# sunchao/leveldb-rs

Measured on AMD Instinct MI355X. Metric: GiB/s device-resident batched CRC32C, 4KiB blocks; %HBM-peak at 1/2/4/8 GPUs, higher is better.
Workload: dtype u32

## Files before the change

leveldb-rs_amd/csrc/blocks.hip:

```cpp
#include <hip/hip_runtime.h>

#include <algorithm>
#include <string>

#include "lvh.h"

namespace lvk {

template <int G, bool STRIDED>
__global__ __launch_bounds__(kThreads) void crc32c_batch_kernel(Params P, const uint4 *__restrict__ image) {
    if (static_cast<uint64_t>(blockIdx.x) * kWaves * (64 / G) >= P.n) return;
    stage_tables(image);
    const uint32_t lane = threadIdx.x & 63u;
    const uint32_t wave = threadIdx.x >> 6;
    const Lut L = make_lut(lane);
    constexpr uint32_t kGroups = 64 / G;
    const uint64_t gid = (static_cast<uint64_t>(blockIdx.x) * kWaves + wave) * kGroups + lane / G;
    const uint64_t gstride = static_cast<uint64_t>(gridDim.x) * kWaves * kGroups;
    group_stream<G, STRIDED>(P, gid, gstride, lane % G, L);
}

constexpr uint32_t kFuseMax = 16;

__device__ __forceinline__ void fuse_pieces(const Params &P, const uint32_t *fm, uint32_t (&res)[kWaves][64],
                                            uint32_t lane, uint32_t wave) {
    __syncthreads();
    if (wave != 0) return;
    const uint32_t s = 1u << P.pshift;
    const uint64_t v = static_cast<uint64_t>(blockIdx.x) * 64u + lane;
    const uint32_t k = lane & (s - 1u);
    uint32_t acc = v < P.n ? gf2_apply(fm + (s - 1u - k) * 33u, res[lane >> 2][lane & 3u]) : 0u;
    for (uint32_t d = s >> 1; d >= 1; d >>= 1) acc ^= __shfl_xor(acc, d);
    if (v < P.n && k == 0) P.out[v >> P.pshift] = final_crc(P, acc);
}
static_assert(kFuseMax * 33 <= kWaves * 64, "fused combine matrices fit g_oidx");
template <int G, bool SEEDED, bool PIECES = false, bool FUSE = false, bool GATHER = false>
__global__ __launch_bounds__(kThreads) void crc32c_blocks_kernel(Params P, uint32_t nb,
                                                                 const uint4 *__restrict__ image) {
    static_assert(!FUSE || (PIECES && G == 16), "fused combine: pieces of the G = 16 kernel");
    const uint32_t lane = threadIdx.x & 63u;
    const uint32_t wave = __builtin_amdgcn_readfirstlane(threadIdx.x >> 6);
    constexpr uint32_t kGroups = 64 / G;
    constexpr uint64_t kRow = 16ull * G;
    constexpr uint64_t kBatch = kRow * U;
    const uint32_t gl = lane % G;
    constexpr uint32_t kW = kWaves;
    uint64_t blk = (static_cast<uint64_t>(blockIdx.x) * kW + wave) * kGroups + lane / G;
    const uint64_t gstride = static_cast<uint64_t>(gridDim.x) * kW * kGroups;
    const uint64_t wblk0 = (static_cast<uint64_t>(blockIdx.x) * kW + wave) * kGroups;
    const uint64_t pmask = (1ull << P.pshift) - 1;
    auto block_off = [&](uint64_t k) -> uint64_t {
        const uint64_t kk = k < P.n ? k : 0;
        const uint64_t b = PIECES ? kk >> P.pshift : kk;
        if constexpr (GATHER) return P.off[b];
        return b * P.stride;
    };
    auto report = [&](uint32_t bad) {
        if constexpr (GATHER)
            if (bad && P.herr) atomicOr(P.herr, bad);
    };
    auto block_at = [&](uint64_t k, uint64_t bo) {
        const uint64_t kk = k < P.n ? k : 0;
        if constexpr (GATHER) bo &= ~static_cast<uint64_t>(15);
        if constexpr (PIECES) return P.base + bo + (kk & pmask) * P.plen + 16u * gl;
        return P.base + bo + 16u * gl;
    };
    auto block_ptr = [&](uint64_t k) { return block_at(k, block_off(k)); };
    auto seed_ld = [&](uint64_t k) -> uint32_t {
        const uint64_t kk = k < P.n ? k : 0;
        if constexpr (PIECES) {
            const uint32_t sd = SEEDED ? ~P.seed[kk >> P.pshift] : 0xffffffffu;
            return (kk & pmask) ? 0u : sd;
        }
        return ~P.seed[kk];
    };
    constexpr bool kVarS0 = SEEDED || PIECES;

    const uint64_t o0 = block_off(blk);
    uint64_t ptr = block_at(blk, o0);
    uint64_t o1 = GATHER ? block_off(blk + gstride) : 0;
    uint64_t o2 = o1;
    uint32_t s0 = kVarS0 ? seed_ld(blk) : 0xffffffffu;
    uint32_t s0n = s0;
    uint4 slot0[U], slot1[U];
#pragma unroll
    for (uint32_t i = 0; i < U; ++i) slot0[i] = load16(ptr + kRow * i);
    const uint64_t nblk = PIECES ? (P.n >> P.pshift) : P.n;
    const uint64_t lstr = static_cast<uint64_t>(gridDim.x) * kThreads;
    const uint64_t lb0 = static_cast<uint64_t>(blockIdx.x) * kThreads + threadIdx.x;
    uint32_t lq[4] = {0, 0, 0, 0};
    const bool lcheck = GATHER && P.herr;
    if (lcheck) {
#pragma unroll
        for (uint32_t i = 0; i < 4; ++i) {
            const uint64_t b = lb0 + i * lstr;
            lq[i] = b < nblk ? P.len[b] ^ P.hlen : 0u;
        }
    }
    uint32_t *const fm = &g_oidx[0][0];
    if constexpr (FUSE) {
        const uint32_t nw = (1u << P.pshift) * 32u;
        for (uint32_t i = threadIdx.x; i < nw; i += kThreads) fm[(i >> 5) * 33 + (i & 31u)] = P.mats[i];
    }
    stage_tables(image);
    uint32_t lbad = lq[0] | lq[1] | lq[2] | lq[3];
    if (lcheck)
        for (uint64_t b = lb0 + 4 * lstr; b < nblk; b += lstr) lbad |= P.len[b] ^ P.hlen;
    if constexpr (GATHER) report(((o0 & 15u) ? LV_HINT_ERR_MISALIGNED : 0u) | (lbad ? LV_HINT_ERR_NOT_UNIFORM : 0u));
    if (wblk0 >= P.n) {
        if constexpr (FUSE) fuse_pieces(P, fm, g_ocrc, lane, wave);
        return;
    }
    if constexpr (PIECES) {
        if (nb <= U && (FUSE || wblk0 + gstride >= P.n)) {
            uint4 v1[U], v2[U], v3[U];
#pragma unroll
            for (uint32_t i = 0; i < U; ++i) {
                v1[i] = load16(ptr + kBatch * (nb > 1 ? 1u : 0u) + kRow * i);
                v2[i] = load16(ptr + kBatch * (nb > 2 ? 2u : 0u) + kRow * i);
                v3[i] = load16(ptr + kBatch * (nb > 3 ? 3u : 0u) + kRow * i);
            }
            const Lut L = make_lut(lane);
            uint32_t A[U] = {};
            if (gl == 0) slot0[0].x ^= kVarS0 ? seed_ld(blk) : 0xffffffffu;
            fold_batch_carry(slot0, A, L, nb == 1);
            if (nb > 1) fold_batch_carry(v1, A, L, nb == 2);
            if (nb > 2) fold_batch_carry(v2, A, L, nb == 3);
            if (nb > 3) fold_batch_carry(v3, A, L, nb == 4);
            const uint32_t X = merge_group<G, -1, -1, true>(A, L);
            if constexpr (FUSE) {
                if (gl == 0) g_ocrc[wave][lane / G] = X;
                fuse_pieces(P, fm, g_ocrc, lane, wave);
            } else {
                if (gl == 0 && blk < P.n) P.out[blk] = X;
            }
            return;
        }
    }
    const uint64_t rounds = (P.n - 1 - wblk0) / gstride + 1;
    if (G == 16 && nb >= 8 && rounds * nb >= 64)
        for (uint32_t k = 0; k < wave * LVK_STAGGER; ++k) __builtin_amdgcn_s_sleep(32);
    const Lut L = make_lut(lane);
    uint32_t A[U] = {};
    uint32_t st_val = 0;
    uint64_t st_ptr = 0;

    auto step = [&](uint64_t r, uint32_t j, uint4(&cur)[U], uint4(&nxt)[U]) {
        const bool lastj = j + 1 == nb;
        const bool more = !lastj || r + 1 < rounds;
        if constexpr (GATHER) o2 = block_off(blk + 2 * gstride);
        const uint64_t nptr = lastj ? (GATHER ? block_at(blk + gstride, o1) : block_ptr(blk + gstride)) : ptr + kBatch;
        const uint64_t lptr = more ? nptr : GATHER ? ptr : P.base + 16u * gl;
        if constexpr (kVarS0) s0n = seed_ld(blk + gstride);
#pragma unroll
        for (uint32_t i = 0; i < U; ++i) nxt[i] = load16(lptr + kRow * i);
        if (j == 0 && gl == 0) cur[0].x ^= s0;
        fold_batch_carry(cur, A, L, lastj);
        if (lastj) {
            const uint32_t X = merge_group<G, -1, -1, true>(A, L);
#pragma unroll
            for (uint32_t i = 0; i < U; ++i) A[i] = 0u;
            if (gl == 0) g_ocrc[wave][(r % G) * kGroups + lane / G] = PIECES ? X : final_crc(P, X);
            if (!FUSE && ((r + 1) % G == 0 || r + 1 == rounds)) {
                __builtin_amdgcn_wave_barrier();
                const uint64_t r0 = r - r % G;
                const uint64_t k = wblk0 + (r0 + lane / kGroups) * gstride + lane % kGroups;
                st_val = g_ocrc[wave][lane];
                st_ptr = reinterpret_cast<uint64_t>(P.out + (k < P.n ? k : 0));
                if (lane < (r - r0 + 1) * kGroups && k < P.n) *reinterpret_cast<uint32_t *>(st_ptr) = st_val;
                __builtin_amdgcn_wave_barrier();
            }
            blk += gstride;
            if constexpr (kVarS0) s0 = s0n;
            if constexpr (GATHER) {
                if (o1 & 15u) report(LV_HINT_ERR_MISALIGNED);
                o1 = o2;
            }
        }
        ptr = nptr;
    };

    const uint64_t total = rounds * nb;
    uint64_t t = 0;
    uint64_t r = 0;
    uint32_t j = 0;
    for (;;) {
        step(r, j, slot0, slot1);
        if (++t == total) break;
        if (++j == nb) { j = 0; ++r; }
        step(r, j, slot1, slot0);
        if (++t == total) break;
        if (++j == nb) { j = 0; ++r; }
    }
    asm volatile("" ::"v"(st_val), "v"(st_ptr));
    if constexpr (FUSE) fuse_pieces(P, fm, g_ocrc, lane, wave);
}

__global__ __launch_bounds__(256) void combine_pieces_kernel(const uint32_t *__restrict__ raw, uint64_t n, uint32_t s,
                                                             const uint32_t *__restrict__ mats,
                                                             uint32_t *__restrict__ out, uint32_t flags) {
    __shared__ uint32_t M[65 * 33];
    for (uint32_t i = threadIdx.x; i < 65 * 32; i += blockDim.x) M[(i >> 5) * 33 + (i & 31u)] = mats[i];
    __syncthreads();
    const uint32_t lane = threadIdx.x & 63u;
    const uint32_t w = s < 64 ? s : 64, reps = s <= 64 ? 1 : s / 64;
    const uint64_t nw = static_cast<uint64_t>(gridDim.x) * (blockDim.x / 64);
    for (uint64_t b = static_cast<uint64_t>(blockIdx.x) * (blockDim.x / 64) + (threadIdx.x >> 6); b < n; b += nw) {
        uint32_t acc = 0;
        if (lane < w) {
            uint32_t nx = raw[b * s + lane];
            for (uint32_t m = 0; m < reps; ++m) {
                const uint32_t cur = nx;
                if (m + 1 < reps) nx = raw[b * s + lane + 64 * (m + 1)];
                acc = (m ? gf2_apply(M + 64 * 33, acc) : 0u) ^ cur;
            }
            acc = gf2_apply(M + (w - 1 - lane) * 33, acc);
        }
#pragma unroll
        for (int k = 32; k >= 1; k >>= 1) acc ^= __shfl_xor(acc, k);
        if (lane == 0) {
            const uint32_t crc = ~acc;
            out[b] = (flags & LV_CRC_MASK) ? mask_crc(crc) : crc;
        }
    }
}

__global__ __launch_bounds__(1024) void combine_pieces_wg_kernel(const uint32_t *__restrict__ raw, uint32_t s,
                                                                 const uint32_t *__restrict__ tabs,
                                                                 uint32_t *__restrict__ out, uint32_t flags) {
    __shared__ __attribute__((aligned(16))) uint32_t T[11 * 1024];
    __shared__ uint32_t part[16];
    const uint32_t c = s / 1024u;
    const uint32_t lc = c >= 4u ? 2u : 1u;
    stage_words(T, tabs, 256u);
    stage_words(T + 1024, tabs + lc * 1024u, 10u * 256u);
    __syncthreads();
    const uint32_t t = threadIdx.x, lane = t & 63u, w = t >> 6;
    const uint64_t b = blockIdx.x;
    uint32_t acc = 0;
    for (uint32_t i = 0; i < c; ++i) acc = (i ? tab_shift(T, acc) : 0u) ^ raw[b * s + t * c + i];
#pragma unroll
    for (uint32_t u = 0; u < 6; ++u) {
        const uint32_t right = __shfl_down(acc, 1u << u);
        const uint32_t sh = tab_shift(T + (1u + u) * 1024u, acc);
        if ((lane & ((2u << u) - 1u)) == 0) acc = sh ^ right;
    }
    if (lane == 0) part[w] = acc;
    __syncthreads();
    if (w == 0) {
        acc = lane < 16u ? part[lane] : 0u;
#pragma unroll
        for (uint32_t u = 0; u < 4; ++u) {
            const uint32_t right = __shfl_down(acc, 1u << u);
            const uint32_t sh = tab_shift(T + (7u + u) * 1024u, acc);
            if ((lane & ((2u << u) - 1u)) == 0) acc = sh ^ right;
        }
        if (lane == 0) {
            const uint32_t crc = ~acc;
            out[b] = (flags & LV_CRC_MASK) ? mask_crc(crc) : crc;
        }
    }
}

}

namespace lvh {

template <int G, bool STRIDED>
void launch_one(const DevCtx &c, int gi, const uint8_t *arena, const uint64_t *off,
                const uint32_t *len, uint64_t stride, uint32_t blen, const uint32_t *seed,
                uint32_t *out, uint64_t n, uint32_t flags, hipStream_t s) {
    const uint64_t groups_per_wg = static_cast<uint64_t>(lvk::kWaves) * (64 / G);
    uint64_t grid = (n + groups_per_wg - 1) / groups_per_wg;
    if (grid > static_cast<uint64_t>(c.cus)) grid = c.cus;
    if (grid == 0) grid = 1;
    lvk::Params P{};
    P.base = reinterpret_cast<uint64_t>(arena);
    P.off = off;
    P.len = len;
    P.seed = seed;
    P.out = out;
    P.n = n;
    P.stride = stride;
    P.blen = blen;
    P.flags = flags;
    P.ent = nullptr;
    P.sseed = nullptr;
    static const std::string name = std::string("crc32c_batch_kernel<") + std::to_string(G) +
                                    (STRIDED ? ",strided>" : ",offsets>");
    g_kernel = name.c_str();
    hipLaunchKernelGGL((lvk::crc32c_batch_kernel<G, STRIDED>), dim3(static_cast<uint32_t>(grid)),
                       dim3(lvk::kThreads), 0, s, P, c.image[gi]);
}

template <bool STRIDED>
void launch_g(const DevCtx &c, int gi, const uint8_t *arena, const uint64_t *off,
              const uint32_t *len, uint64_t stride, uint32_t blen, const uint32_t *seed,
              uint32_t *out, uint64_t n, uint32_t flags, hipStream_t s) {
    switch (gi) {
        case 0: launch_one<1, STRIDED>(c, gi, arena, off, len, stride, blen, seed, out, n, flags, s); break;
        case 1: launch_one<4, STRIDED>(c, gi, arena, off, len, stride, blen, seed, out, n, flags, s); break;
        case 2: launch_one<16, STRIDED>(c, gi, arena, off, len, stride, blen, seed, out, n, flags, s); break;
        default: launch_one<64, STRIDED>(c, gi, arena, off, len, stride, blen, seed, out, n, flags, s); break;
    }
}

void launch_group(const DevCtx &c, bool strided, int gi, const uint8_t *arena, const uint64_t *off,
                  const uint32_t *len, uint64_t stride, uint32_t blen, const uint32_t *seed, uint32_t *out, uint64_t n,
                  uint32_t flags, hipStream_t s) {
    if (strided)
        launch_g<true>(c, gi, arena, off, len, stride, blen, seed, out, n, flags, s);
    else
// ... 194 lines not shown
```

leveldb-rs_amd/csrc/context.hip:

```cpp
#include <hip/hip_runtime.h>

#include <algorithm>
#include <cstring>
#include <thread>

#include "../../include/lvgpu/crc32c.h"
#include "crc32c_gf2.h"
#include "lvh.h"

namespace lvk {

__device__ __forceinline__ uint64_t splitmix64(uint64_t x) {
    x += 0x9E3779B97F4A7C15ull;
    x = (x ^ (x >> 30)) * 0xBF58476D1CE4E5B9ull;
    x = (x ^ (x >> 27)) * 0x94D049BB133111EBull;
    return x ^ (x >> 31);
}

__global__ void fill_words_kernel(uint64_t *dst, uint64_t word0, uint64_t nwords, uint64_t seed) {
    for (uint64_t i = blockIdx.x * 256ull + threadIdx.x; i < nwords; i += gridDim.x * 256ull)
        dst[i] = splitmix64(seed ^ (word0 + i));
}

__global__ void fill_bytes_kernel(uint8_t *dst, uint64_t begin, uint64_t nbytes, uint64_t seed) {
    for (uint64_t i = blockIdx.x * 256ull + threadIdx.x; i < nbytes; i += gridDim.x * 256ull) {
        const uint64_t k = begin + i;
        dst[i] = static_cast<uint8_t>(splitmix64(seed ^ (k >> 3)) >> (8 * (k & 7)));
    }
}

}

namespace lvh {

thread_local std::string g_err;
thread_local const char *g_kernel = "";

int set_err(int code, const std::string &msg) {
    g_err = msg;
    return code;
}

const std::vector<uint32_t> &host_image(int gi) {
    static std::vector<uint32_t> images[kImages];
    static std::once_flag once;
    std::call_once(once, [] {
        uint32_t T[4][256], C[6][4][256];
        lvgpu::slice_tables(T);
        for (int k = 0; k < 6; ++k) lvgpu::shift_tables(16ull << k, C[k]);
        for (int i = 0; i < 4; ++i) {
            const uint64_t G = static_cast<uint64_t>(kGs[i]);
            uint32_t W4[4][256], W1[4][256], W2[4][256];
            lvgpu::shift_tables(16ull * G * lvk::U, W4);
            lvgpu::shift_tables(16ull * G, W1);
            lvgpu::shift_tables(32ull * G, W2);
            std::vector<uint32_t> &im = images[i];
            im.assign(lvk::kImageWords, 0u);
            uint32_t *ra = &im[lvk::kRegionA / 4], *rb = &im[lvk::kRegionB / 4];
            for (int e = 0; e < 256; ++e)
                for (int c = 0; c < 8; ++c)
                    for (int k = 0; k < 4; ++k) {
                        ra[e * 64 + 4 * c + k] = T[k][e];
                        ra[e * 64 + 32 + 4 * c + k] = W4[3 - k][e];
                        rb[e * 64 + 4 * c + k] = W1[3 - k][e];
                        rb[e * 64 + 32 + 4 * c + k] = W2[3 - k][e];
                    }
            uint32_t *rc = &im[lvk::kComb / 4];
            for (int k = 0; k < 6; ++k)
                for (int j = 0; j < 4; ++j)
                    for (int e = 0; e < 256; ++e) rc[(k * 4 + j) * 256 + e] = C[k][j][e];
        }
        uint32_t WT[4][256];
        lvgpu::shift_tables(256ull * lvk::kSstRows, WT);
        images[kTableImage] = images[2];
        uint32_t *ra = &images[kTableImage][lvk::kRegionA / 4];
        for (int e = 0; e < 256; ++e)
            for (int c = 0; c < 8; ++c)
                for (int k = 0; k < 4; ++k) ra[e * 64 + 32 + 4 * c + k] = WT[3 - k][e];
        for (int i = 0; i < 4; ++i) {
            uint32_t J[4][256];
            lvgpu::shift_tables(16ull * kGs[i] * lvk::U - 12, J);
            images[kBlocksImage + i] = images[i];
            uint32_t *rj = &images[kBlocksImage + i][lvk::kRegionA / 4];
            for (int e = 0; e < 256; ++e)
                for (int c = 0; c < 8; ++c)
                    for (int k = 0; k < 4; ++k) rj[e * 64 + 32 + 4 * c + k] = J[3 - k][e];
        }
    });
    return images[gi];
}

DevCounters g_count[64];

DevCounters &counters() {
    int d = 0;
    if (hipGetDevice(&d) != hipSuccess || d < 0 || d >= 64) d = 0;
    return g_count[d];
}

int grow_dev(uint8_t **p, size_t *cap, size_t need) {
    if (*cap >= need) return 0;
    if (*p) LV_HIP(hipFree(*p));
    *p = nullptr;
    *cap = 0;
    LV_HIP(hipMalloc(p, need));
    counters().allocs++;
    *cap = need;
    return 0;
}

int grow_pinned(uint8_t **p, size_t *cap, size_t need) {
    if (*cap >= need) return 0;
    if (*p) LV_HIP(hipHostFree(*p));
    *p = nullptr;
    *cap = 0;
    LV_HIP(hipHostMalloc(p, need, hipHostMallocDefault));
    counters().allocs++;
    *cap = need;
    return 0;
}

bool is_pinned(const void *p) {
    hipPointerAttribute_t a;
    const hipError_t e = hipPointerGetAttributes(&a, p);
    if (e != hipSuccess) {
        (void)hipGetLastError();
        return false;
    }
    return a.type == hipMemoryTypeHost;
}

void par_memcpy(uint8_t *dst, const uint8_t *src, size_t bytes, unsigned threads) {
    unsigned nt = std::thread::hardware_concurrency();
    nt = nt == 0 ? 1 : (nt > threads ? threads : nt);
    if (bytes < (4u << 20) || nt == 1) {
        std::memcpy(dst, src, bytes);
        return;
    }
    std::vector<std::thread> th;
    const size_t per = (bytes + nt - 1) / nt;
    for (unsigned t = 0; t < nt; ++t) {
        const size_t lo = t * per;
        if (lo >= bytes) break;
        const size_t len = bytes - lo < per ? bytes - lo : per;
        th.emplace_back([=] { std::memcpy(dst + lo, src + lo, len); });
    }
    for (auto &x : th) x.join();
}

DevCtx g_dev[64];

int current_ctx(DevCtx **out) {
    int dev = 0;
    hipError_t e = hipGetDevice(&dev);
    if (e != hipSuccess) return set_err(LV_ERR_NO_DEVICE, std::string("hipGetDevice: ") + hipGetErrorString(e));
    if (dev < 0 || dev >= 64) return set_err(LV_ERR_NO_DEVICE, "device index out of range");
    DevCtx &c = g_dev[dev];
    std::lock_guard<std::mutex> lk(c.m);
    if (!c.ready) {
        hipDeviceProp_t prop;
        LV_HIP(hipGetDeviceProperties(&prop, dev));
        c.cus = prop.multiProcessorCount;
        for (int i = 0; i < kImages; ++i) {
            const auto &im = host_image(i);
            LV_HIP(hipMalloc(&c.image[i], im.size() * 4));
            counters().allocs++;
            LV_HIP(hipMemcpy(c.image[i], im.data(), im.size() * 4, hipMemcpyHostToDevice));
        }
        {
            std::vector<uint32_t> bt(lvk::kBaseMats * 1024);
            for (uint32_t i = 0; i < lvk::kBaseMats; ++i) {
                uint32_t S[4][256];
                lvgpu::shift_tables(1ull << i, S);
                for (int j = 0; j < 4; ++j)
                    for (int e = 0; e < 256; ++e) bt[i * 1024 + j * 256 + e] = S[j][e];
            }
            LV_HIP(hipMalloc(&c.base_tabs, bt.size() * 4));
            counters().allocs++;
            LV_HIP(hipMemcpy(c.base_tabs, bt.data(), bt.size() * 4, hipMemcpyHostToDevice));
        }
        c.ready = true;
    }
    *out = &c;
    return 0;
}

int pick_gi(uint64_t len) {
    if (len <= 128) return 0;
    if (len <= 1024) return 1;
    if (len <= 16384) return 2;
    return 3;
}

int forced_gi(uint32_t flags) {
    const uint32_t f = (flags & LV_CRC_GROUP_MASK) >> 8;
    return f ? static_cast<int>(f) - 1 : -1;
}

static StreamWs *find_ws(DevCtx &c, hipStream_t s, bool create) {
    std::lock_guard<std::mutex> mk(c.ws_m);
    if (!create) {
        auto it = c.ws.find(s);
        return it == c.ws.end() ? nullptr : it->second.get();
    }
    auto &slot = c.ws[s];
    if (!slot) slot.reset(new StreamWs);
    return slot.get();
}

int stream_ws_bytes(DevCtx &c, hipStream_t s, size_t need, uint8_t **out, std::unique_lock<std::mutex> *lk) {
    StreamWs *w = find_ws(c, s, true);
    *lk = std::unique_lock<std::mutex>(w->m);
    if (w->cap < need) {
        if (w->p) LV_HIP(hipFree(w->p));
        w->p = nullptr;
        w->cap = 0;
        LV_HIP(hipMalloc(&w->p, need));
        counters().allocs++;
        w->cap = need;
    }
    *out = w->p;
    return 0;
}

int stream_ws(DevCtx &c, hipStream_t s, uint64_t n, uint8_t **out, std::unique_lock<std::mutex> *lk) {
    return stream_ws_bytes(c, s, sort_ws_bytes(n), out, lk);
}

int stream_err(DevCtx &c, hipStream_t s, uint32_t **out) {
    StreamWs *w = find_ws(c, s, true);
    std::lock_guard<std::mutex> lk(w->em);
    if (!w->err) {
        LV_HIP(hipHostMalloc(reinterpret_cast<void **>(&w->herr), 4, hipHostMallocDefault));
        LV_HIP(hipMalloc(&w->err, 4));
        counters().allocs += 2;
        LV_HIP(hipMemsetAsync(w->err, 0, 4, s));
    }
    *out = w->err;
    return 0;
// ... 340 lines not shown
```

leveldb-rs_amd/csrc/lvk/core.h:

```cpp
#pragma once
#include <hip/hip_runtime.h>

#include <cstdint>

#include "../../../include/lvgpu/crc32c.h"
#include "knobs.h"

namespace lvk {

constexpr int kThreads = 1024;
constexpr int kWaves = kThreads / 64;
constexpr uint32_t U = 4;

constexpr uint32_t kRegionA = 0;
constexpr uint32_t kRegionB = 65536;
constexpr uint32_t kHalf = 128;
constexpr uint32_t kComb = 131072;
constexpr int kImageWords = (131072 + 6 * 4 * 1024) / 4;

static __shared__ __attribute__((aligned(16))) uint32_t g_lds[kImageWords];

static __shared__ uint32_t g_oidx[kWaves][64];
static __shared__ uint32_t g_ocrc[kWaves][64];
static_assert(sizeof(uint32_t) * (kImageWords + 2 * kWaves * 64) <= 163840, "LDS budget");

struct Lut {
    uint32_t lv, sel0, sel1, sel2, sel3;
};

__device__ __forceinline__ Lut make_lut(uint32_t lane) {
    const uint32_t g = lane & 31u, c = g & 7u, q = g >> 3;
    Lut L;
    L.lv = 0;
    uint32_t sel[4];
#pragma unroll
    for (uint32_t i = 0; i < 4; ++i) {
        const uint32_t k = (q + i) & 3u;
        L.lv |= ((4u * c + k) * 4u) << (8u * i);
        sel[i] = 0x0C0C0000u | ((4u + 3u - k) << 8) | i;
    }
    L.sel0 = sel[0];
    L.sel1 = sel[1];
    L.sel2 = sel[2];
    L.sel3 = sel[3];
    return L;
}

__device__ __forceinline__ uint32_t lds_word(uint32_t byte_addr) {
    return *reinterpret_cast<const uint32_t *>(reinterpret_cast<const char *>(g_lds) + byte_addr);
}

__device__ __forceinline__ uint32_t xor3(uint32_t a, uint32_t b, uint32_t c) {
    return __builtin_amdgcn_bitop3_b32(a, b, c, 0x96);
}

template <uint32_t OFF>
__device__ __forceinline__ uint32_t lookup4(uint32_t s, const Lut &L) {
    const uint32_t a0 = __builtin_amdgcn_perm(s, L.lv, L.sel0);
    const uint32_t a1 = __builtin_amdgcn_perm(s, L.lv, L.sel1);
    const uint32_t a2 = __builtin_amdgcn_perm(s, L.lv, L.sel2);
    const uint32_t a3 = __builtin_amdgcn_perm(s, L.lv, L.sel3);
    return xor3(lds_word(a0 + OFF), lds_word(a1 + OFF), lds_word(a2 + OFF)) ^ lds_word(a3 + OFF);
}

template <uint32_t OFF>
__device__ __forceinline__ uint32_t lookup4x(uint32_t s, uint32_t x, const Lut &L) {
    const uint32_t a0 = __builtin_amdgcn_perm(s, L.lv, L.sel0);
    const uint32_t a1 = __builtin_amdgcn_perm(s, L.lv, L.sel1);
    const uint32_t a2 = __builtin_amdgcn_perm(s, L.lv, L.sel2);
    const uint32_t a3 = __builtin_amdgcn_perm(s, L.lv, L.sel3);
    return xor3(xor3(lds_word(a0 + OFF), lds_word(a1 + OFF), lds_word(a2 + OFF)), lds_word(a3 + OFF), x);
}

__device__ __forceinline__ uint32_t r0_granule(uint4 v, const Lut &L) {
    uint32_t s = lookup4x<kRegionA>(v.x, v.y, L);
    s = lookup4x<kRegionA>(s, v.z, L);
    s = lookup4x<kRegionA>(s, v.w, L);
    return lookup4<kRegionA>(s, L);
}

template <int I>
__device__ __forceinline__ uint32_t lut_addr(uint32_t s, const Lut &L) {
    const uint32_t sel = I == 0 ? L.sel0 : I == 1 ? L.sel1 : I == 2 ? L.sel2 : L.sel3;
    return __builtin_amdgcn_perm(s, L.lv, sel);
}

__device__ __forceinline__ uint32_t comb_shift(uint32_t a, int k) {
    const uint32_t *t = g_lds + (kComb / 4) + k * 1024;
    return t[a & 0xffu] ^ t[256 + ((a >> 8) & 0xffu)] ^ t[512 + ((a >> 16) & 0xffu)] ^
           t[768 + (a >> 24)];
}

template <bool FIRST, int W4K = -1, uint32_t NU = U, uint32_t W4OFF = kRegionA + kHalf, uint32_t SKIP = 0>
__device__ __forceinline__ void fold_batch(const uint4 (&v)[NU], uint32_t (&A)[NU], const Lut &L) {
    static_assert(SKIP == 0 || FIRST, "only a first batch skips rows");
    static_assert(SKIP < NU, "at least one row");
    uint32_t s[NU], w[NU], w3[NU];
#pragma unroll
    for (uint32_t i = 0; i < NU; ++i) s[i] = v[i].x;
    if constexpr (SKIP > 0) {
#pragma unroll
        for (uint32_t i = 0; i < SKIP; ++i) A[i] = 0u;
    }
    if constexpr (!FIRST && W4K >= 0) {
#pragma unroll
        for (uint32_t i = 0; i < NU; ++i) {
            w[i] = comb_shift(A[i], W4K);
            w3[i] = 0u;
        }
    } else if constexpr (!FIRST) {
        uint32_t aa[NU][4];
#pragma unroll
        for (uint32_t i = 0; i < NU; ++i) {
            aa[i][0] = lut_addr<0>(A[i], L);
            aa[i][1] = lut_addr<1>(A[i], L);
            aa[i][2] = lut_addr<2>(A[i], L);
            aa[i][3] = lut_addr<3>(A[i], L);
        }
#pragma unroll
        for (uint32_t i = 0; i < NU; ++i) {
            w[i] = xor3(lds_word(aa[i][0] + W4OFF), lds_word(aa[i][1] + W4OFF),
                        lds_word(aa[i][2] + W4OFF));
            w3[i] = lds_word(aa[i][3] + W4OFF);
        }
    }
#pragma unroll
    for (uint32_t step = 0; step < 4; ++step) {
        uint32_t ad[NU][4];
#pragma unroll
        for (uint32_t i = SKIP; i < NU; ++i) {
            ad[i][0] = lut_addr<0>(s[i], L);
            ad[i][1] = lut_addr<1>(s[i], L);
            ad[i][2] = lut_addr<2>(s[i], L);
            ad[i][3] = lut_addr<3>(s[i], L);
        }
        uint32_t t[NU][4];
#pragma unroll
        for (uint32_t i = SKIP; i < NU; ++i)
#pragma unroll
            for (uint32_t k = 0; k < 4; ++k) t[i][k] = lds_word(ad[i][k] + kRegionA);
#pragma unroll
        for (uint32_t i = SKIP; i < NU; ++i) {
            const uint32_t x = xor3(t[i][0], t[i][1], t[i][2]);
            if (step < 3) {
                const uint32_t nw = step == 0 ? v[i].y : step == 1 ? v[i].z : v[i].w;
                s[i] = xor3(x, t[i][3], nw);
            } else if constexpr (FIRST) {
                A[i] = x ^ t[i][3];
            } else {
                A[i] = x ^ xor3(t[i][3], w[i], w3[i]);
            }
        }
    }
}

template <uint32_t NU = U>
__device__ __forceinline__ void fold_batch_carry(const uint4 (&v)[NU], uint32_t (&A)[NU], const Lut &L, bool last) {
    Lut L3 = L;
    L3.lv = last ? L.lv : L.lv | 0x80808080u;
    uint32_t s[NU];
#pragma unroll
    for (uint32_t i = 0; i < NU; ++i) s[i] = v[i].x ^ A[i];
#pragma unroll
    for (uint32_t step = 0; step < 4; ++step) {
        const Lut &Ls = step < 3 ? L : L3;
        uint32_t ad[NU][4];
#pragma unroll
        for (uint32_t i = 0; i < NU; ++i) {
            ad[i][0] = lut_addr<0>(s[i], Ls);
            ad[i][1] = lut_addr<1>(s[i], Ls);
            ad[i][2] = lut_addr<2>(s[i], Ls);
            ad[i][3] = lut_addr<3>(s[i], Ls);
        }
        uint32_t t[NU][4];
#pragma unroll
        for (uint32_t i = 0; i < NU; ++i)
#pragma unroll
            for (uint32_t k = 0; k < 4; ++k) t[i][k] = lds_word(ad[i][k] + kRegionA);
#pragma unroll
        for (uint32_t i = 0; i < NU; ++i) {
            const uint32_t x = xor3(t[i][0], t[i][1], t[i][2]);
            if (step < 3) {
                const uint32_t nw = step == 0 ? v[i].y : step == 1 ? v[i].z : v[i].w;
                s[i] = xor3(x, t[i][3], nw);
            } else {
                A[i] = x ^ t[i][3];
            }
        }
    }
}

__device__ __forceinline__ uint32_t byte_step(uint32_t s, uint32_t b) {
    const uint32_t c4 = (__lane_id() & 7u) * 4u;
    const uint32_t e = (s ^ b) & 0xffu;
    return g_lds[e * 64u + c4] ^ (s >> 8);
}

__device__ __forceinline__ uint32_t fix_word(uint32_t w, int32_t rel, uint32_t s0) {
    const int32_t z = -rel;
    const uint32_t keep = z <= 0 ? 0xffffffffu : (z >= 4 ? 0u : 0xffffffffu << (8 * z));
    const uint32_t sx =
        (rel >= 4 || rel <= -4) ? 0u : (rel >= 0 ? s0 >> (8 * rel) : s0 << (8 * z));
    return (w & keep) ^ sx;
}

typedef uint32_t u32x4 __attribute__((ext_vector_type(4)));
typedef const __attribute__((address_space(1))) u32x4 g_u32x4;

__device__ __forceinline__ uint4 to_uint4(u32x4 v) { return make_uint4(v.x, v.y, v.z, v.w); }

__device__ __forceinline__ uint4 load16(uint64_t addr) {
    return to_uint4(__builtin_nontemporal_load(reinterpret_cast<g_u32x4 *>(addr)));
}

__device__ __forceinline__ uint4 load16_rt(uint64_t addr) {
    return to_uint4(*reinterpret_cast<g_u32x4 *>(addr));
}

template <uint32_t I>
__device__ __forceinline__ uint4 load_row(uint64_t addr) {
    if constexpr (I == U - 1) return load16_rt(addr);
    return load16(addr);
}

__device__ __forceinline__ uint32_t mask_crc(uint32_t c) {
    return ((c >> 15) | (c << 17)) + 0xa282ead8u;
}

struct Params {
    uint64_t base;
    const uint64_t *off;
    const uint32_t *len;
    const uint32_t *seed;
    uint32_t *out;
    uint64_t n;
    uint64_t stride;
    uint32_t blen;
    uint32_t flags;
    uint64_t plen;
    uint32_t pshift;
    const uint4 *ent;
    const uint32_t *sseed;
    uint64_t nplain;
    uint32_t *part;
    uint32_t *tmp;
    const uint32_t *mats;
    const uint32_t *tabs;
    uint32_t hident;
    uint32_t *herr;
    uint64_t htotal;
    uint32_t hlen;
    uint32_t huni;
};

struct Geo {
    uint64_t abase;
    uint32_t bid;
    uint32_t len;
    uint32_t seed;
    uint32_t nb;
    int32_t hoff;
    uint32_t alow;
};

template <int G>
__device__ __forceinline__ Geo make_geo(uint64_t a, uint32_t len, uint32_t seed) {
    constexpr int32_t GU = G * static_cast<int32_t>(U);
    Geo q;
    q.abase = a & ~static_cast<uint64_t>(15);
    q.len = len;
    q.seed = seed;
    const uint32_t alow = static_cast<uint32_t>(a & 15u);
    const int32_t ng = static_cast<int32_t>(((alow + len) >> 4));
    const int32_t nb = ng > 0 ? (ng + GU - 1) / GU : 1;
    q.nb = static_cast<uint32_t>(nb);
    q.hoff = ng - GU * nb;
    const bool fix2 = nb > 1 && q.hoff == -(GU - 1) && alow > 12u;
    q.alow = alow | (fix2 ? 16u : 0u);
    return q;
}

template <int G, bool STRIDED>
__device__ __forceinline__ Geo fetch_geo(const Params &P, uint64_t i) {
    Geo q;
    uint64_t b = i;
    if constexpr (STRIDED) {
        q = make_geo<G>(P.base + b * P.stride, P.blen, P.seed ? P.seed[b] : 0u);
    } else if (P.ent) {
        const uint4 e = P.ent[i];
        b = e.w;
        q = make_geo<G>(P.base + ((static_cast<uint64_t>(e.y) << 32) | e.x), e.z, P.seed ? P.seed[b] : 0u);
    } else {
        q = make_geo<G>(P.base + P.off[b], P.len[b], P.seed ? P.seed[b] : 0u);
    }
    q.bid = static_cast<uint32_t>(b);
    return q;
}

template <int G>
__device__ __forceinline__ void load_batch(const Geo &q, uint32_t j, uint32_t gl, uint4 (&v)[U]) {
    const int32_t d = q.hoff + static_cast<int32_t>(G * U * j + gl);
    const uint64_t p = q.abase + (static_cast<int64_t>(d) << 4);
    v[0] = load_row<0>(p);
    v[1] = load_row<1>(p + 16u * G);
    v[2] = load_row<2>(p + 32u * G);
    v[3] = load_row<3>(p + 48u * G);
}

template <int G>
__device__ __forceinline__ void load_batch0(const Geo &q, uint32_t gl, uint4 (&v)[U]) {
#pragma unroll
    for (uint32_t i = 0; i < U; ++i) {
        int32_t d = q.hoff + static_cast<int32_t>(G * i + gl);
        d = d < 0 ? 0 : d;
        const uint64_t a = q.abase + (static_cast<uint32_t>(d) << 4);
        v[i] = i == U - 1 ? load16_rt(a) : load16(a);
    }
}

__device__ __forceinline__ uint4 load_tail(const Geo &q, uint32_t gl) {
    const uint32_t end = (q.alow & 15u) + q.len;
    if (gl == 0 && (end & 15u)) return load16(q.abase + (end & ~15u));
    return make_uint4(0, 0, 0, 0);
}

template <int G>
__device__ __forceinline__ void fix_head(const Geo &q, uint32_t j, uint32_t gl, uint4 (&v)[U]) {
    const uint32_t s0 = q.len >= 4 ? ~q.seed : 0u;
    const int32_t alow = static_cast<int32_t>(q.alow & 15u);
#pragma unroll
    for (uint32_t i = 0; i < U; ++i) {
        const int32_t d = q.hoff + static_cast<int32_t>(G * (U * j + i) + gl);
        if (d == 0 || (d == 1 && alow > 12)) {
            const int32_t rel = d * 16 - alow;
            v[i].x = fix_word(v[i].x, rel, s0);
            v[i].y = fix_word(v[i].y, rel + 4, s0);
            v[i].z = fix_word(v[i].z, rel + 8, s0);
            v[i].w = fix_word(v[i].w, rel + 12, s0);
        }
    }
}

// ... 14 lines not shown
    for (int k = 0; (1 << k) < G; ++k) {
        const uint32_t other = __shfl_down(X, 1u << k, G);
        X = comb_shift(X, k) ^ other;
    }
    const uint32_t alow = q.alow & 15u;
    const uint32_t end = alow + q.len;
    if (gl == 0 && ((end & 15u) != 0 || q.len < 4)) {
        const uint32_t tb = end & ~15u;
        const uint32_t hi = end - tb;
        const uint32_t lo = alow > tb ? alow - tb : 0u;
        const uint32_t s0 = q.len >= 4 ? ~q.seed : 0u;
        const uint32_t tw[4] = {tail.x, tail.y, tail.z, tail.w};
        for (uint32_t i = lo; i < hi; ++i) {
            uint32_t by = (tw[i >> 2] >> (8u * (i & 3u))) & 0xffu;
            const uint32_t rel = tb + i - alow;
            if (rel < 4) by ^= (s0 >> (8u * rel)) & 0xffu;
            X = byte_step(X, by);
        }
        if (q.len < 4) {
            uint32_t s = ~q.seed;
            for (uint32_t i = 0; i < q.len; ++i) s = byte_step(s, 0u);
            X ^= s;
        }
    }
    if (gl == 0) {
        const uint32_t crc = ~X;
        P.out[q.bid] = (P.flags & LV_CRC_MASK) ? mask_crc(crc) : crc;
    }
}

template <int G>
struct Stream {
    Geo q, qn;
    uint64_t b;
    uint4 tail;
    uint32_t A[U];
    uint32_t j;
};

template <int G, bool STRIDED>
__device__ __forceinline__ bool stream_step(const Params &P, uint64_t gstride, uint32_t gl, const Lut &L,
                                            Stream<G> &S, uint4 (&cur)[U], uint4 (&nxt)[U]) {
    const bool last = S.j + 1 == S.q.nb;
    const bool has_next = S.b + gstride < P.n;
    if (!last)
        load_batch<G>(S.q, S.j + 1, gl, nxt);
    else if (has_next)
        load_batch0<G>(S.qn, gl, nxt);
    if (S.j == 0)
        fix_head<G>(S.q, 0, gl, cur);
    else if (S.j == 1 && (S.q.alow & 16u))
        fix_head<G>(S.q, 1, gl, cur);
    fold_batch<false>(cur, S.A, L);
    if (S.j == 0) drop_pre_rows<G>(S.q, gl, S.A);
    if (!last) {
        ++S.j;
        return false;
    }
    finish<G>(P, S.q, S.A, S.tail, gl, L);
#pragma unroll
    for (uint32_t i = 0; i < U; ++i) S.A[i] = 0u;
    if (!has_next) return true;
    S.b += gstride;
    S.q = S.qn;
    S.tail = load_tail(S.q, gl);
    if (S.b + gstride < P.n) S.qn = fetch_geo<G, STRIDED>(P, S.b + gstride);
    S.j = 0;
    return false;
}

template <int G, bool STRIDED>
__device__ __forceinline__ void group_stream(const Params &P, uint64_t gid, uint64_t gstride,
                                             uint32_t gl, const Lut &L) {
    if (gid >= P.n) return;
    Stream<G> S;
#pragma unroll
    for (uint32_t i = 0; i < U; ++i) S.A[i] = 0u;
    S.b = gid;
    S.q = fetch_geo<G, STRIDED>(P, S.b);
    if (gid + gstride < P.n) S.qn = fetch_geo<G, STRIDED>(P, gid + gstride);
    S.tail = load_tail(S.q, gl);
    S.j = 0;
    uint4 cur[U], nxt[U];
    load_batch0<G>(S.q, gl, cur);
    if constexpr (G == 1) {
        for (;;) {
            if (stream_step<G, STRIDED>(P, gstride, gl, L, S, cur, nxt)) break;
            if (stream_step<G, STRIDED>(P, gstride, gl, L, S, nxt, cur)) break;
        }
    } else {
        for (;;) {
            if (stream_step<G, STRIDED>(P, gstride, gl, L, S, cur, nxt)) break;
#pragma unroll
            for (uint32_t i = 0; i < U; ++i) cur[i] = nxt[i];
        }
    }
}

__device__ __forceinline__ void stage_tables(const uint4 *__restrict__ image) {
    constexpr int kVec = kImageWords / 4;
    constexpr int kPer = (kVec + kThreads - 1) / kThreads;
    uint4 *l4 = reinterpret_cast<uint4 *>(g_lds);
    g_u32x4 *src = reinterpret_cast<g_u32x4 *>(reinterpret_cast<uint64_t>(image));
    u32x4 r[kPer];
#pragma unroll
    for (int k = 0; k < kPer; ++k) {
        const int i = threadIdx.x + k * kThreads;
        if (i < kVec) r[k] = src[i];
    }
#pragma unroll
    for (int k = 0; k < kPer; ++k) {
        const int i = threadIdx.x + k * kThreads;
        if (i < kVec) l4[i] = to_uint4(r[k]);
    }
    __syncthreads();
}

template <int G, bool DPP>
__device__ __forceinline__ uint32_t lanes_down(uint32_t x, int k) {
    if constexpr (DPP) {
        switch (k) {
        case 0: return __builtin_amdgcn_mov_dpp(x, 0x101, 0xf, 0xf, true);
        case 1: return __builtin_amdgcn_mov_dpp(x, 0x102, 0xf, 0xf, true);
        case 2: return __builtin_amdgcn_mov_dpp(x, 0x104, 0xf, 0xf, true);
        case 3: return __builtin_amdgcn_mov_dpp(x, 0x108, 0xf, 0xf, true);
        default: break;
        }
    }
    return __shfl_down(x, 1u << k, G);
}

template <int G, int W1K = -1, int W2K = -1, bool DPP = false>
__device__ __forceinline__ uint32_t merge_group(const uint32_t (&A)[U], const Lut &L) {
    uint32_t x01, x23, X;
    if constexpr (W1K >= 0) {
        x01 = comb_shift(A[0], W1K) ^ A[1];
        x23 = comb_shift(A[2], W1K) ^ A[3];
    } else {
        x01 = lookup4<kRegionB>(A[0], L) ^ A[1];
        x23 = lookup4<kRegionB>(A[2], L) ^ A[3];
    }
    if constexpr (W2K >= 0)
        X = comb_shift(x01, W2K) ^ x23;
    else
        X = lookup4<kRegionB + kHalf>(x01, L) ^ x23;
#pragma unroll
    for (int k = 0; (1 << k) < G; ++k) {
        const uint32_t other = lanes_down<G, DPP>(X, k);
        X = comb_shift(X, k) ^ other;
    }
    return X;
}

__device__ __forceinline__ uint32_t final_crc(const Params &P, uint32_t X) {
    const uint32_t crc = ~X;
    return (P.flags & LV_CRC_MASK) ? mask_crc(crc) : crc;
}

__device__ __forceinline__ uint32_t gf2_apply(const uint32_t *m, uint32_t v) {
    uint32_t r = 0;
#pragma unroll
    for (int j = 0; j < 32; ++j) r ^= (v >> j & 1u) ? m[j] : 0u;
    return r;
}

constexpr uint32_t kPow2Tabs = 13;

__device__ __forceinline__ uint32_t tab_shift(const uint32_t *t, uint32_t a) {
    return t[a & 0xffu] ^ t[256 + ((a >> 8) & 0xffu)] ^ t[512 + ((a >> 16) & 0xffu)] ^ t[768 + (a >> 24)];
}

__device__ __forceinline__ void stage_words(uint32_t *dst, const uint32_t *src, uint32_t n4) {
    const uint4 *s4 = reinterpret_cast<const uint4 *>(src);
    uint4 *d4 = reinterpret_cast<uint4 *>(dst);
    const uint32_t b = blockDim.x;
    uint32_t i = threadIdx.x;
    for (; i + 3u * b < n4; i += 4u * b) {
        const uint4 v0 = s4[i], v1 = s4[i + b], v2 = s4[i + 2u * b], v3 = s4[i + 3u * b];
        d4[i] = v0;
        d4[i + b] = v1;
        d4[i + 2u * b] = v2;
        d4[i + 3u * b] = v3;
    }
    for (; i < n4; i += b) d4[i] = s4[i];
}

constexpr uint32_t kBaseMats = 48;

constexpr uint32_t kSstRows = LVK_SST_ROWS;
static_assert(kSstRows == 3 || kSstRows == 4, "table walk: 3 or 4 rows per batch");
constexpr uint32_t kSealRows = LVK_SEAL_ROWS;
static_assert(kSealRows == kSstRows || kSealRows == 4, "seal: the table image's rows, or 4 on the G = 16 image");

}
```

Before: 6246.

## Fold group-merge shifts into last-step tables and join groups via DPP

The final byte-slice step of each block now uses per-lane position-specific tables in region B, so the shift each row needs is folded into the last lookup. The per-group merge becomes a DPP row-shift XOR tree with only a few combine-table lookups, replacing the log-depth merge_group with its per-level comb_shift. New host-side tables for region B and the combine region are built per group size. The intent is to cut LDS lookups and serial shuffle depth in the reduction; the risk is correctness across group sizes and extra table setup.

New measurement: 6319 (median of 6 runs). 1.2% higher.

```diff
diff --git a/leveldb-rs_amd/csrc/blocks.hip b/leveldb-rs_amd/csrc/blocks.hip
--- a/leveldb-rs_amd/csrc/blocks.hip
+++ b/leveldb-rs_amd/csrc/blocks.hip
@@ -127,7 +127,7 @@
             if (nb > 1) fold_batch_carry(v1, A, L, nb == 2);
             if (nb > 2) fold_batch_carry(v2, A, L, nb == 3);
             if (nb > 3) fold_batch_carry(v3, A, L, nb == 4);
-            const uint32_t X = merge_group<G, -1, -1, true>(A, L);
+            const uint32_t X = join_group<G>(A, lane);
             if constexpr (FUSE) {
                 if (gl == 0) g_ocrc[wave][lane / G] = X;
                 fuse_pieces(P, fm, g_ocrc, lane, wave);
@@ -155,9 +155,13 @@
 #pragma unroll
         for (uint32_t i = 0; i < U; ++i) nxt[i] = load16(lptr + kRow * i);
         if (j == 0 && gl == 0) cur[0].x ^= s0;
-        fold_batch_carry(cur, A, L, lastj);
-        if (lastj) {
-            const uint32_t X = merge_group<G, -1, -1, true>(A, L);
+        uint32_t sl[U];
+        carry_slices(cur, A, L, sl);
+        if (!lastj) {
+            carry_finish<false>(sl, A, L);
+        } else {
+            carry_finish<true>(sl, A, L);
+            const uint32_t X = join_group<G>(A, lane);
 #pragma unroll
             for (uint32_t i = 0; i < U; ++i) A[i] = 0u;
             if (gl == 0) g_ocrc[wave][(r % G) * kGroups + lane / G] = PIECES ? X : final_crc(P, X);
diff --git a/leveldb-rs_amd/csrc/context.hip b/leveldb-rs_amd/csrc/context.hip
--- a/leveldb-rs_amd/csrc/context.hip
+++ b/leveldb-rs_amd/csrc/context.hip
@@ -85,6 +85,28 @@
             for (int e = 0; e < 256; ++e)
                 for (int c = 0; c < 8; ++c)
                     for (int k = 0; k < 4; ++k) rj[e * 64 + 32 + 4 * c + k] = J[3 - k][e];
+            const uint64_t G = static_cast<uint64_t>(kGs[i]), w = G < 8 ? G : 8;
+            uint32_t *rb = &images[kBlocksImage + i][lvk::kRegionB / 4];
+            for (uint64_t c = 0; c < 8; ++c) {
+                uint32_t E0[4][256], E1[4][256];
+                const uint64_t d = 16 * (w - 1 - c % w);
+                lvgpu::shift_tables(4 + d, E0);
+                lvgpu::shift_tables(4 + 32 * G + d, E1);
+                for (int e = 0; e < 256; ++e)
+                    for (int k = 0; k < 4; ++k) {
+                        rb[e * 64 + 4 * c + k] = E0[3 - k][e];
+                        rb[e * 64 + 32 + 4 * c + k] = E1[3 - k][e];
+                    }
+            }
+            static const uint64_t kJoin[4][4] = {{16, 0, 0, 0}, {64, 0, 0, 0}, {128, 256, 384, 0}, {1024, 128, 256, 512}};
+            uint32_t *rc = &images[kBlocksImage + i][lvk::kComb / 4];
+            std::fill(rc, rc + 6 * 1024, 0u);
+            for (int k = 0; k < 4 && kJoin[i][k]; ++k) {
+                uint32_t S[4][256];
+                lvgpu::shift_tables(kJoin[i][k], S);
+                for (int j = 0; j < 4; ++j)
+                    for (int e = 0; e < 256; ++e) rc[(k * 4 + j) * 256 + e] = S[j][e];
+            }
         }
     });
     return images[gi];
diff --git a/leveldb-rs_amd/csrc/lvk/core.h b/leveldb-rs_amd/csrc/lvk/core.h
--- a/leveldb-rs_amd/csrc/lvk/core.h
+++ b/leveldb-rs_amd/csrc/lvk/core.h
@@ -154,40 +154,93 @@
     }
 }
 
+struct LutE {
+    uint32_t lv01, lv23;
+    uint32_t sel0, sel1, sel2, sel3;
+};
+static_assert(kRegionB == 0x10000u, "LutE sets address bit 16");
+
+__device__ __forceinline__ LutE make_lute(const Lut &L) {
+    LutE E;
+    E.lv01 = (L.lv & 0x0000ffffu) | 0x01010000u;
+    E.lv23 = (L.lv & 0xffff0000u) | 0x00000101u;
+    E.sel0 = (L.sel0 & 0xff00ffffu) | 0x00030000u;
+    E.sel1 = (L.sel1 & 0xff00ffffu) | 0x00030000u;
+    E.sel2 = L.sel2 & 0xff00ffffu;
+    E.sel3 = L.sel3 & 0xff00ffffu;
+    return E;
+}
+
+template <uint32_t NU, uint32_t OFF_LO, uint32_t OFF_HI>
+__device__ __forceinline__ void carry_last_step(const uint32_t (&s)[NU], uint32_t (&A)[NU], uint32_t lv01,
+                                                uint32_t lv23, uint32_t sel0, uint32_t sel1, uint32_t sel2,
+                                                uint32_t sel3) {
+    uint32_t ad[NU][4];
+#pragma unroll
+    for (uint32_t i = 0; i < NU; ++i) {
+        ad[i][0] = __builtin_amdgcn_perm(s[i], lv01, sel0);
+        ad[i][1] = __builtin_amdgcn_perm(s[i], lv01, sel1);
+        ad[i][2] = __builtin_amdgcn_perm(s[i], lv23, sel2);
+        ad[i][3] = __builtin_amdgcn_perm(s[i], lv23, sel3);
+    }
+    uint32_t t[NU][4];
+#pragma unroll
+    for (uint32_t i = 0; i < NU; ++i)
+#pragma unroll
+        for (uint32_t k = 0; k < 4; ++k) t[i][k] = lds_word(ad[i][k] + (i < NU / 2 ? OFF_LO : OFF_HI));
+#pragma unroll
+    for (uint32_t i = 0; i < NU; ++i) A[i] = xor3(t[i][0], t[i][1], t[i][2]) ^ t[i][3];
+}
+
+template <uint32_t NU = U>
+__device__ __forceinline__ void carry_slices(const uint4 (&v)[NU], const uint32_t (&A)[NU], const Lut &L,
+                                             uint32_t (&s)[NU]) {
+#pragma unroll
+    for (uint32_t i = 0; i < NU; ++i) s[i] = v[i].x ^ A[i];
+#pragma unroll
+    for (uint32_t step = 0; step < 3; ++step) {
+        uint32_t ad[NU][4];
+#pragma unroll
+        for (uint32_t i = 0; i < NU; ++i) {
+            ad[i][0] = lut_addr<0>(s[i], L);
+            ad[i][1] = lut_addr<1>(s[i], L);
+            ad[i][2] = lut_addr<2>(s[i], L);
+            ad[i][3] = lut_addr<3>(s[i], L);
+        }
+        uint32_t t[NU][4];
+#pragma unroll
+        for (uint32_t i = 0; i < NU; ++i)
+#pragma unroll
+            for (uint32_t k = 0; k < 4; ++k) t[i][k] = lds_word(ad[i][k] + kRegionA);
+#pragma unroll
+        for (uint32_t i = 0; i < NU; ++i) {
+            const uint32_t nw = step == 0 ? v[i].y : step == 1 ? v[i].z : v[i].w;
+            s[i] = xor3(xor3(t[i][0], t[i][1], t[i][2]), t[i][3], nw);
+        }
+    }
+}
+
+template <bool LAST, uint32_t NU = U>
+__device__ __forceinline__ void carry_finish(const uint32_t (&s)[NU], uint32_t (&A)[NU], const Lut &L) {
+    static_assert(NU == U, "region B positions the four rows of a batch");
+    if constexpr (LAST) {
+        const LutE E = make_lute(L);
+        carry_last_step<NU, kRegionB - 0x10000u + kHalf, kRegionB - 0x10000u>(s, A, E.lv01, E.lv23, E.sel0, E.sel1,
+                                                                              E.sel2, E.sel3);
+    } else {
+        const uint32_t lvj = L.lv | 0x80808080u;
+        carry_last_step<NU, kRegionA, kRegionA>(s, A, lvj, lvj, L.sel0, L.sel1, L.sel2, L.sel3);
+    }
+}
+
 template <uint32_t NU = U>
 __device__ __forceinline__ void fold_batch_carry(const uint4 (&v)[NU], uint32_t (&A)[NU], const Lut &L, bool last) {
-    Lut L3 = L;
-    L3.lv = last ? L.lv : L.lv | 0x80808080u;
     uint32_t s[NU];
-#pragma unroll
-    for (uint32_t i = 0; i < NU; ++i) s[i] = v[i].x ^ A[i];
-#pragma unroll
-    for (uint32_t step = 0; step < 4; ++step) {
-        const Lut &Ls = step < 3 ? L : L3;
-        uint32_t ad[NU][4];
-#pragma unroll
-        for (uint32_t i = 0; i < NU; ++i) {
-            ad[i][0] = lut_addr<0>(s[i], Ls);
-            ad[i][1] = lut_addr<1>(s[i], Ls);
-            ad[i][2] = lut_addr<2>(s[i], Ls);
-            ad[i][3] = lut_addr<3>(s[i], Ls);
-        }
-        uint32_t t[NU][4];
-#pragma unroll
-        for (uint32_t i = 0; i < NU; ++i)
-#pragma unroll
-            for (uint32_t k = 0; k < 4; ++k) t[i][k] = lds_word(ad[i][k] + kRegionA);
-#pragma unroll
-        for (uint32_t i = 0; i < NU; ++i) {
-            const uint32_t x = xor3(t[i][0], t[i][1], t[i][2]);
-            if (step < 3) {
-                const uint32_t nw = step == 0 ? v[i].y : step == 1 ? v[i].z : v[i].w;
-                s[i] = xor3(x, t[i][3], nw);
-            } else {
-                A[i] = x ^ t[i][3];
-            }
-        }
-    }
+    carry_slices(v, A, L, s);
+    if (last)
+        carry_finish<true>(s, A, L);
+    else
+        carry_finish<false>(s, A, L);
 }
 
 __device__ __forceinline__ uint32_t byte_step(uint32_t s, uint32_t b) {
@@ -508,6 +561,56 @@
     return X;
 }
 
+template <uint32_t N>
+__device__ __forceinline__ uint32_t row_up(uint32_t x) {
+    return __builtin_amdgcn_mov_dpp(x, 0x100 + N, 0xf, 0xf, true);
+}
+template <uint32_t N>
+__device__ __forceinline__ uint32_t row_down(uint32_t x) {
+    return __builtin_amdgcn_mov_dpp(x, 0x110 + N, 0xf, 0xf, true);
+}
+
+__device__ __forceinline__ uint32_t comb_shift_at(uint32_t a, uint32_t tb) {
+    return xor3(lds_word(tb + (a & 0xffu) * 4u), lds_word(tb + 1024u + ((a >> 8) & 0xffu) * 4u),
+                lds_word(tb + 2048u + ((a >> 16) & 0xffu) * 4u)) ^
+           lds_word(tb + 3072u + (a >> 24) * 4u);
+}
+
+template <int G>
+__device__ __forceinline__ uint32_t join_group(const uint32_t (&A)[U], uint32_t lane) {
+    const uint32_t y = A[0] ^ A[2], z = A[1] ^ A[3];
+    if constexpr (G == 1) {
+        return comb_shift_at(y, kComb) ^ z;
+    } else {
+        const uint32_t yp = y ^ row_up<1>(y), zp = z ^ row_down<1>(z);
+        uint32_t q = (lane & 1u) ? zp : yp;
+        q ^= row_up<2>(q);
+        if constexpr (G >= 8) q ^= row_up<4>(q);
+        if constexpr (G == 16) {
+            const uint32_t gl = lane & 15u;
+            const bool part = gl <= 1u || gl == 8u;
+            const uint32_t tb = kComb + (gl == 0u ? 2u * 4096u : gl == 8u ? 4096u : 0u);
+            uint32_t r = comb_shift_at(part ? q : 0u, tb);
+            r ^= row_up<1>(r);
+            r ^= row_up<8>(r);
+            return r ^ row_up<9>(q);
+        } else {
+            constexpr uint32_t w = G < 8 ? G : 8;
+            const bool first = (lane & (w - 1u)) == 0u;
+            uint32_t X = comb_shift_at(first ? q : 0u, kComb) ^ row_up<1>(q);
+            if constexpr (G == 64) {
+                X = first ? X : 0u;
+#pragma unroll
+                for (int k = 0; k < 3; ++k) {
+                    const uint32_t other = lanes_down<G, true>(X, 3 + k);
+                    X = comb_shift_at(X, kComb + (1u + k) * 4096u) ^ other;
+                }
+            }
+            return X;
+        }
+    }
+}
+
 __device__ __forceinline__ uint32_t final_crc(const Params &P, uint32_t X) {
     const uint32_t crc = ~X;
     return (P.flags & LV_CRC_MASK) ? mask_crc(crc) : crc;
```
